# microsoft/ORBIT-Dataset

Measured on AMD Instinct MI355X. Metric: query frames/sec per task (224×224, 5-way ProtoNet) + frame accuracy vs ref, higher is better.
Workload: dtype f32

## Files before the change

### orbit-dataset_amd/csrc/pw_stream.hip

```cpp
#include <algorithm>
#include <type_traits>
#include "common.h"
#include "se_gate.h"

namespace orbit {

using f32x4 = __attribute__((ext_vector_type(4))) float;

struct PwsParams {
    const float* x;
    const float* w;
    float* y;
    const float* scale;
    const float* shift;
    const float* residual;
    const float* partial;
    const float *w1, *b1, *w2t, *b2;
    float* gate_out;
    float inv_hw;
    int KT, chunks, R, HW, Cout;
    int tiles;
    int bpf;
};

template <int KC, int NG, int TP>
__global__ __launch_bounds__(256) void pw_stream_kernel(PwsParams p) {
    constexpr int K = 16 * KC;
    extern __shared__ __attribute__((aligned(16))) float sm[];
    f32x4* wl = reinterpret_cast<f32x4*>(sm);
    float* gl = sm + KC * NG * 256;
    float* sg = gl + K;
    const int tid = threadIdx.x, lane = tid & 63, wave = tid >> 6;
    const int q = lane >> 4;
    const int b = blockIdx.x / p.bpf, seg = blockIdx.x - b * p.bpf;
    const int t_beg = (int)((long)seg * p.tiles / p.bpf), t_end = (int)((long)(seg + 1) * p.tiles / p.bpf);
    const size_t pix0 = (size_t)b * p.HW + (lane & 15);
    const bool has_res = p.residual != nullptr;

    auto has = [&](int s) { return t_beg + (4 * s + wave) * TP < t_end; };
    auto tile_of = [&](int s, int u) { return t_beg + (4 * s + wave) * TP + u; };
    auto row_of = [&](int s, int u) {
        const int t = tile_of(s, u);
        return pix0 + (size_t)16 * (t < t_end ? t : tile_of(s, 0));
    };

    f32x4 xa[TP][KC];
    if (has(0)) {
#pragma unroll
        for (int u = 0; u < TP; ++u) {
            const float* px = p.x + row_of(0, u) * K + 4 * q;
#pragma unroll
            for (int c = 0; c < KC; ++c) xa[u][c] = *reinterpret_cast<const f32x4*>(px + 16 * c);
        }
    }

    for (int i = tid; i < KC * NG * 64; i += 256) {
        const int l = i & 63, g = (i >> 6) % NG, c = (i >> 6) / NG;
        wl[i] = *reinterpret_cast<const f32x4*>(p.w + (size_t)(16 * g + (l & 15)) * p.KT + 16 * c + 4 * (l >> 4));
    }
    se_gate_frame<256, 4>(p.partial + (size_t)b * p.chunks * K, p.chunks, p.inv_hw, p.w1, p.b1, p.w2t, p.b2, gl, K, p.R,
                          nullptr, sg);
    __syncthreads();
    if (p.gate_out != nullptr && seg == 0)
        for (int c4 = tid; c4 < K / 4; c4 += 256)
            reinterpret_cast<f32x4*>(p.gate_out + (size_t)b * K)[c4] = reinterpret_cast<const f32x4*>(gl)[c4];

    f32x4 sc[NG], sh[NG];
#pragma unroll
    for (int g = 0; g < NG; ++g) {
        const int ch = 16 * g + 4 * q;
        const bool ok = ch < p.Cout;
        sc[g] = ok ? *reinterpret_cast<const f32x4*>(p.scale + ch) : (f32x4){0.f, 0.f, 0.f, 0.f};
        sh[g] = ok ? *reinterpret_cast<const f32x4*>(p.shift + ch) : (f32x4){0.f, 0.f, 0.f, 0.f};
    }

    auto step = [&](int s, auto refill) {
        constexpr bool REFILL = decltype(refill)::value;
        __asm__ volatile("" ::: "memory");
        size_t row[TP], nrow[TP];
#pragma unroll
        for (int u = 0; u < TP; ++u) row[u] = row_of(s, u), nrow[u] = REFILL ? row_of(s + 1, u) : row[u];
        f32x4 rr[TP][NG];
        if (has_res)
#pragma unroll
            for (int u = 0; u < TP; ++u)
#pragma unroll
                for (int g = 0; g < NG; ++g) {
                    const int ch = 16 * g + 4 * q;
                    rr[u][g] = *reinterpret_cast<const f32x4*>(p.residual + row[u] * p.Cout + (ch < p.Cout ? ch : 0));
                }
        f32x4 acc[TP][NG];
#pragma unroll
        for (int u = 0; u < TP; ++u)
#pragma unroll
            for (int g = 0; g < NG; ++g) acc[u][g] = (f32x4){0.f, 0.f, 0.f, 0.f};
#pragma unroll
        for (int c = 0; c < KC; ++c) {
            const f32x4 gv = *reinterpret_cast<const f32x4*>(gl + 16 * c + 4 * q);
            f32x4 xv[TP];
#pragma unroll
            for (int u = 0; u < TP; ++u) {
                xv[u] = xa[u][c] * gv;
                if (REFILL) xa[u][c] = *reinterpret_cast<const f32x4*>(p.x + nrow[u] * K + 4 * q + 16 * c);
            }
#pragma unroll
            for (int g = 0; g < NG; ++g) {
                const f32x4 wv = wl[(c * NG + g) * 64 + lane];
#pragma unroll
                for (int e = 0; e < 4; ++e)
#pragma unroll
                    for (int u = 0; u < TP; ++u)
                        acc[u][g] = __builtin_amdgcn_mfma_f32_16x16x4f32(wv[e], xv[u][e], acc[u][g], 0, 0, 0);
            }
        }
#pragma unroll
        for (int u = 0; u < TP; ++u) {
            if (tile_of(s, u) >= t_end) continue;
#pragma unroll
            for (int g = 0; g < NG; ++g) {
                const int ch = 16 * g + 4 * q;
                if (ch >= p.Cout) continue;
                f32x4 o = acc[u][g] * sc[g] + sh[g];
                if (has_res) o += rr[u][g];
                *reinterpret_cast<f32x4*>(p.y + row[u] * p.Cout + ch) = o;
            }
        }
    };
    int s = 0;
    for (; has(s + 1); ++s) step(s, std::true_type{});
    if (has(s)) step(s, std::false_type{});
}

namespace {
struct PwsVariant {
    int kc, ng, tp;
    void (*fn)(PwsParams);
};
const PwsVariant kVariants[] = {
    {2, 1, 2, pw_stream_kernel<2, 1, 2>},
    {6, 2, 1, pw_stream_kernel<6, 2, 1>},
    {9, 2, 1, pw_stream_kernel<9, 2, 1>},
    {9, 3, 1, pw_stream_kernel<9, 3, 1>},
};
const PwsVariant* find_variant(int Cin, int Cout) {
    if (Cin % 16 != 0 || Cout % 8 != 0 || Cout > 48) return nullptr;
    for (const PwsVariant& v : kVariants)
        if (v.kc == Cin / 16 && v.ng == cdiv(Cout, 16)) return &v;
    return nullptr;
}
}

bool pw_stream_supported(int Cin, int Cout, int H, int W) {
    return find_variant(Cin, Cout) != nullptr && (H * W) % 16 == 0;
}

int launch_pw_stream(const PwStreamDesc& d, hipStream_t s) {
    ORBIT_REQUIRE(d.x && d.w_packed && d.y && d.scale && d.shift && d.partial && d.w1 && d.b1 && d.w2t && d.b2,
                  "pw_stream: null pointer");
    ORBIT_REQUIRE(pw_stream_supported(d.Cin, d.Cout, d.H, d.W), "pw_stream: unsupported layer %d -> %d @%dx%d", d.Cin, d.Cout,
                  d.H, d.W);
    ORBIT_REQUIRE(d.B > 0 && d.chunks > 0 && d.se_hw > 0 && d.R > 0, "pw_stream: bad sizes");
    const PwsVariant& v = *find_variant(d.Cin, d.Cout);
    const ConvPackGeom geom = conv_pack_geom(d.Cin, d.Cout, 1, 1, 0);
    ORBIT_REQUIRE(geom.kt >= d.Cin && geom.cout_pad >= 16 * v.ng, "pw_stream: packed filter too small");
    PwsParams p;
    p.x = d.x, p.w = d.w_packed, p.y = d.y, p.scale = d.scale, p.shift = d.shift, p.residual = d.residual;
    p.partial = d.partial, p.w1 = d.w1, p.b1 = d.b1, p.w2t = d.w2t, p.b2 = d.b2, p.gate_out = d.gate_out;
    p.inv_hw = 1.0f / (float)d.se_hw;
    p.KT = geom.kt, p.chunks = d.chunks, p.R = d.R, p.HW = d.H * d.W, p.Cout = d.Cout;
    p.tiles = p.HW / 16;
    p.bpf = std::max(1, std::min(p.tiles, cdiv(p.tiles, 24 * v.tp)));
    ORBIT_REQUIRE((long long)d.B * p.bpf < (1ll << 31), "pw_stream: grid too large");
    const size_t lds = ((size_t)v.kc * v.ng * 256 + d.Cin + ((d.Cin + d.R + 3) & ~3) + 4 * 256) * sizeof(float);
    const double M = (double)d.B * p.HW;
    char name[48];
    snprintf(name, sizeof(name), "conv_pw_stream<%dx%d%s>", d.Cin, d.Cout, d.residual ? ",res" : "");
    const int rec = prof_start(name, 2.0 * M * d.Cin * d.Cout,
                               4.0 * (M * d.Cin + M * d.Cout * (d.residual ? 2.0 : 1.0) + (double)d.B * d.chunks * d.Cin), s);
    hipLaunchKernelGGL(v.fn, dim3((unsigned)(d.B * p.bpf)), dim3(256), lds, s, p);
    prof_stop(rec, s);
    ORBIT_LAUNCH_CHECK();
    return ORBIT_OK;
}

}

extern "C" {

int orbit_pw_stream_supported(int Cin, int Cout, int H, int W) { return orbit::pw_stream_supported(Cin, Cout, H, W) ? 1 : 0; }

int orbit_op_pw_stream(const float* x, const float* w, const float* scale, const float* shift, const float* residual,
                       const float* partial, int chunks, const float* w1, const float* b1, const float* w2t, const float* b2,
                       int R, float* y, float* gate_out, int B, int H, int W, int Cin, int Cout, orbit_stream_t stream) {
    using namespace orbit;
    ORBIT_REQUIRE(x && w && scale && shift && partial && w1 && b1 && w2t && b2 && y, "op_pw_stream: null pointer");
    hipStream_t s = (hipStream_t)stream;
    const bool fused = get_option("conv_rgemm") && pw_stream_supported(Cin, Cout, H, W);
    const size_t nfl = (conv_packed_floats(Cin, Cout, 1, 1, 0) + 63) & ~(size_t)63;
    const size_t ffl = conv_frag_floats(Cin, Cout, 1, 1, 0);
    const size_t gfl = (fused || gate_out) ? 0 : (size_t)B * Cin;
    float* wp = nullptr;
    ORBIT_HIP_CHECK(hipMallocAsync(reinterpret_cast<void**>(&wp), (nfl + ffl + gfl) * sizeof(float), s));
    int rc = conv_pack_weights(w, wp, Cin, Cout, 1, 1, 0, s);
    if (rc == ORBIT_OK && ffl) rc = conv_frag_pack_weights(w, wp + nfl, Cin, Cout, s);
    if (rc == ORBIT_OK && fused) {
        PwStreamDesc d;
        d.x = x, d.w_packed = wp, d.y = y, d.scale = scale, d.shift = shift, d.residual = residual;
        d.partial = partial, d.chunks = chunks, d.se_hw = H * W, d.w1 = w1, d.b1 = b1, d.w2t = w2t, d.b2 = b2, d.R = R;
        d.gate_out = gate_out, d.B = B, d.H = H, d.W = W, d.Cin = Cin, d.Cout = Cout;
        rc = launch_pw_stream(d, s);
    } else if (rc == ORBIT_OK) {
        float* gate = gate_out ? gate_out : wp + nfl + ffl;
        rc = launch_se_gate2(partial, chunks, H * W, w1, b1, w2t, b2, gate, B, Cin, R, s);
        if (rc == ORBIT_OK) {
            ConvDesc d;
            d.x = x, d.w_packed = wp, d.w_frag = ffl ? wp + nfl : nullptr, d.y = y, d.scale = scale, d.shift = shift;
            d.residual = residual, d.gate = gate, d.B = B, d.H = H, d.W = W, d.Cin = Cin, d.Cout = Cout, d.KH = d.KW = 1;
            d.stride = 1, d.pad_t = d.pad_l = 0, d.Ho = H, d.Wo = W, d.act = ORBIT_ACT_NONE, d.pool2 = 0, d.x_nchw = 0;
            rc = launch_conv(d, s);
        }
    }
    (void)hipFreeAsync(wp, s);
    return rc;
}

}
```

### orbit-dataset_amd/csrc/se_gate.h

```cpp
#pragma once
#include "common.h"
#include "device_util.h"

namespace orbit {

using v4f = __attribute__((ext_vector_type(4))) float;

template <int NT, int U>
__device__ __forceinline__ void se_gate_frame(const float* __restrict__ partial, int chunks, float inv_hw,
                                              const float* __restrict__ w1, const float* __restrict__ b1,
                                              const float* __restrict__ w2t, const float* __restrict__ b2,
                                              float* __restrict__ gate, int C, int R, float* __restrict__ pooled_out, float* sm2) {
    v4f* sp4 = reinterpret_cast<v4f*>(sm2);
    float* hid = sm2 + C;
    const int tid = threadIdx.x;
    const int C4 = C >> 2;
    const v4f* part4 = reinterpret_cast<const v4f*>(partial);
    const int parts = C4 <= NT / 2 ? NT / C4 : 1;
    if (parts > 1 && chunks > 8) {
        v4f* tmp = reinterpret_cast<v4f*>(sm2 + ((C + R + 3) & ~3));
        const int q = tid % C4, part = tid / C4;
        if (part < parts) {
            v4f s = {0.f, 0.f, 0.f, 0.f};
#pragma unroll 4
            for (int k = part; k < chunks; k += parts) s += part4[(size_t)k * C4 + q];
            tmp[part * C4 + q] = s;
        }
        __syncthreads();
        if (tid < C4) {
            v4f s = tmp[tid];
            for (int g = 1; g < parts; ++g) s += tmp[g * C4 + tid];
            sp4[tid] = s * inv_hw;
        }
    } else {
        for (int c4 = tid; c4 < C4; c4 += NT) {
            v4f s = {0.f, 0.f, 0.f, 0.f};
#pragma unroll 8
            for (int k = 0; k < chunks; ++k) s += part4[(size_t)k * C4 + c4];
            sp4[c4] = s * inv_hw;
        }
    }
    __syncthreads();
    if (pooled_out != nullptr)
        for (int c4 = tid; c4 < C4; c4 += NT) reinterpret_cast<v4f*>(pooled_out)[c4] = sp4[c4];
    const int lane = tid & 63, wave = tid >> 6;
    const v4f* w14 = reinterpret_cast<const v4f*>(w1);
    for (int r0 = wave; r0 < R; r0 += U * (NT / 64)) {
        float acc[U];
#pragma unroll
        for (int u = 0; u < U; ++u) acc[u] = 0.f;
        for (int cb = 0; cb < C4; cb += 320) {
            v4f wv[U][5], pv[5];
#pragma unroll
            for (int j = 0; j < 5; ++j) {
                const int c4 = cb + lane + 64 * j;
                const bool ok = c4 < C4;
                pv[j] = ok ? sp4[c4] : (v4f){0.f, 0.f, 0.f, 0.f};
#pragma unroll
                for (int u = 0; u < U; ++u) {
                    const int r = r0 + (NT / 64) * u;
                    wv[u][j] = (ok && r < R) ? w14[(size_t)r * C4 + c4] : (v4f){0.f, 0.f, 0.f, 0.f};
                }
            }
#pragma unroll
            for (int u = 0; u < U; ++u)
#pragma unroll
                for (int j = 0; j < 5; ++j) {
                    const v4f t = wv[u][j] * pv[j];
                    acc[u] += (t[0] + t[1]) + (t[2] + t[3]);
                }
        }
#pragma unroll
        for (int u = 0; u < U; ++u) {
            const int r = r0 + (NT / 64) * u;
            const float sum = wave_sum_dpp(acc[u]);
            if (r < R && lane == 0) {
                const float t = sum + b1[r];
                hid[r] = t / (1.0f + expf(-t));
            }
        }
    }
    __syncthreads();
    const v4f* w24 = reinterpret_cast<const v4f*>(w2t);
    for (int c4 = tid; c4 < C4; c4 += NT) {
        v4f a = *reinterpret_cast<const v4f*>(b2 + 4 * c4);
        int r = 0;
        for (; r + 8 <= R; r += 8) {
            v4f wv[8];
#pragma unroll
            for (int u = 0; u < 8; ++u) wv[u] = w24[(size_t)(r + u) * C4 + c4];
#pragma unroll
            for (int u = 0; u < 8; ++u) a += wv[u] * hid[r + u];
        }
        for (; r < R; ++r) a += w24[(size_t)r * C4 + c4] * hid[r];
        v4f g;
#pragma unroll
        for (int q = 0; q < 4; ++q) g[q] = 1.0f / (1.0f + expf(-a[q]));
        reinterpret_cast<v4f*>(gate)[c4] = g;
    }
}

}
```

Measured before the change: 37360.

## Issue pw_stream prologue loads early and pick blocks-per-frame from occupancy

```diff
diff --git a/orbit-dataset_amd/csrc/pw_stream.hip b/orbit-dataset_amd/csrc/pw_stream.hip
--- a/orbit-dataset_amd/csrc/pw_stream.hip
+++ b/orbit-dataset_amd/csrc/pw_stream.hip
@@ -23,13 +23,16 @@
     int bpf;
 };
 
+constexpr int pws_waves(int KC) { return KC == 2 ? 5 : 4; }
+
 template <int KC, int NG, int TP>
-__global__ __launch_bounds__(256) void pw_stream_kernel(PwsParams p) {
+__global__ __launch_bounds__(256) __attribute__((amdgpu_waves_per_eu(pws_waves(KC)))) void pw_stream_kernel(PwsParams p) {
     constexpr int K = 16 * KC;
     extern __shared__ __attribute__((aligned(16))) float sm[];
     f32x4* wl = reinterpret_cast<f32x4*>(sm);
     float* gl = sm + KC * NG * 256;
-    float* sg = gl + K;
+    f32x4* ssl = reinterpret_cast<f32x4*>(gl + K);
+    float* sg = gl + K + 32 * NG;
     const int tid = threadIdx.x, lane = tid & 63, wave = tid >> 6;
     const int q = lane >> 4;
     const int b = blockIdx.x / p.bpf, seg = blockIdx.x - b * p.bpf;
@@ -44,6 +47,17 @@
         return pix0 + (size_t)16 * (t < t_end ? t : tile_of(s, 0));
     };
 
+    constexpr int NW = (KC * NG * 64 + 255) / 256;
+    f32x4 wq[NW];
+#pragma unroll
+    for (int j = 0; j < NW; ++j) {
+        const int i = tid + 256 * j < KC * NG * 64 ? tid + 256 * j : 0;
+        const int l = i & 63, g = (i >> 6) % NG, c = (i >> 6) / NG;
+        wq[j] = *reinterpret_cast<const f32x4*>(p.w + (size_t)(16 * g + (l & 15)) * p.KT + 16 * c + 4 * (l >> 4));
+    }
+    const int sch = 4 * (tid % (4 * NG)) < p.Cout ? 4 * (tid % (4 * NG)) : 0;
+    const f32x4 ssq = *reinterpret_cast<const f32x4*>((tid < 4 * NG ? p.scale : p.shift) + sch);
+    const SeGateLoads<4> gq = se_gate_request<256, 4, K>(p.w1, p.b1, p.w2t, p.b2, p.R);
     f32x4 xa[TP][KC];
     if (has(0)) {
 #pragma unroll
@@ -53,26 +67,15 @@
             for (int c = 0; c < KC; ++c) xa[u][c] = *reinterpret_cast<const f32x4*>(px + 16 * c);
         }
     }
-
-    for (int i = tid; i < KC * NG * 64; i += 256) {
-        const int l = i & 63, g = (i >> 6) % NG, c = (i >> 6) / NG;
-        wl[i] = *reinterpret_cast<const f32x4*>(p.w + (size_t)(16 * g + (l & 15)) * p.KT + 16 * c + 4 * (l >> 4));
-    }
-    se_gate_frame<256, 4>(p.partial + (size_t)b * p.chunks * K, p.chunks, p.inv_hw, p.w1, p.b1, p.w2t, p.b2, gl, K, p.R,
-                          nullptr, sg);
+#pragma unroll
+    for (int j = 0; j < NW; ++j)
+        if (tid + 256 * j < KC * NG * 64) wl[tid + 256 * j] = wq[j];
+    if (tid < 8 * NG) ssl[tid] = ssq;
+    se_gate_frame_early<256, 4, K>(gq, p.partial + (size_t)b * p.chunks * K, p.chunks, p.inv_hw, gl, p.R, sg);
     __syncthreads();
     if (p.gate_out != nullptr && seg == 0)
         for (int c4 = tid; c4 < K / 4; c4 += 256)
             reinterpret_cast<f32x4*>(p.gate_out + (size_t)b * K)[c4] = reinterpret_cast<const f32x4*>(gl)[c4];
-
-    f32x4 sc[NG], sh[NG];
-#pragma unroll
-    for (int g = 0; g < NG; ++g) {
-        const int ch = 16 * g + 4 * q;
-        const bool ok = ch < p.Cout;
-        sc[g] = ok ? *reinterpret_cast<const f32x4*>(p.scale + ch) : (f32x4){0.f, 0.f, 0.f, 0.f};
-        sh[g] = ok ? *reinterpret_cast<const f32x4*>(p.shift + ch) : (f32x4){0.f, 0.f, 0.f, 0.f};
-    }
 
     auto step = [&](int s, auto refill) {
         constexpr bool REFILL = decltype(refill)::value;
@@ -120,7 +123,7 @@
             for (int g = 0; g < NG; ++g) {
                 const int ch = 16 * g + 4 * q;
                 if (ch >= p.Cout) continue;
-                f32x4 o = acc[u][g] * sc[g] + sh[g];
+                f32x4 o = acc[u][g] * ssl[4 * g + q] + ssl[4 * NG + 4 * g + q];
                 if (has_res) o += rr[u][g];
                 *reinterpret_cast<f32x4*>(p.y + row[u] * p.Cout + ch) = o;
             }
@@ -135,16 +138,45 @@
 struct PwsVariant {
     int kc, ng, tp;
     void (*fn)(PwsParams);
+    size_t occ_lds;
+    int occ;
 };
-const PwsVariant kVariants[] = {
-    {2, 1, 2, pw_stream_kernel<2, 1, 2>},
-    {6, 2, 1, pw_stream_kernel<6, 2, 1>},
-    {9, 2, 1, pw_stream_kernel<9, 2, 1>},
-    {9, 3, 1, pw_stream_kernel<9, 3, 1>},
+PwsVariant kVariants[] = {
+    {2, 1, 2, pw_stream_kernel<2, 1, 2>, 0, 0},
+    {6, 2, 1, pw_stream_kernel<6, 2, 1>, 0, 0},
+    {9, 2, 1, pw_stream_kernel<9, 2, 1>, 0, 0},
+    {9, 3, 1, pw_stream_kernel<9, 3, 1>, 0, 0},
 };
-const PwsVariant* find_variant(int Cin, int Cout) {
+
+long resident_blocks(PwsVariant& v, size_t lds) {
+    static int cus = 0;
+    if (v.occ_lds != lds || cus == 0) {
+        int dev = 0, n = 0;
+        if (hipGetDevice(&dev) != hipSuccess ||
+            hipDeviceGetAttribute(&cus, hipDeviceAttributeMultiprocessorCount, dev) != hipSuccess ||
+            hipOccupancyMaxActiveBlocksPerMultiprocessor(&n, v.fn, 256, lds) != hipSuccess)
+            return 0;
+        v.occ = n, v.occ_lds = lds;
+    }
+    return (long)v.occ * cus;
+}
+
+constexpr int kPrologueBytes = 20 * 1024;
+int blocks_per_frame(int B, int tiles, int K, int tp, long slots) {
+    const double pro = (double)kPrologueBytes / (64.0 * K);
+    int best = 1;
+    double best_cost = 0.0;
+    for (int bpf = 1; bpf <= tiles; ++bpf) {
+        const long rounds = ((long)B * bpf + slots - 1) / slots;
+        const double cost = (double)rounds * (pro + 4 * tp * cdiv(cdiv(tiles, bpf), 4 * tp));
+        if (bpf == 1 || cost < best_cost) best = bpf, best_cost = cost;
+    }
+    return best;
+}
+
+PwsVariant* find_variant(int Cin, int Cout) {
     if (Cin % 16 != 0 || Cout % 8 != 0 || Cout > 48) return nullptr;
-    for (const PwsVariant& v : kVariants)
+    for (PwsVariant& v : kVariants)
         if (v.kc == Cin / 16 && v.ng == cdiv(Cout, 16)) return &v;
     return nullptr;
 }
@@ -160,7 +192,9 @@
     ORBIT_REQUIRE(pw_stream_supported(d.Cin, d.Cout, d.H, d.W), "pw_stream: unsupported layer %d -> %d @%dx%d", d.Cin, d.Cout,
                   d.H, d.W);
     ORBIT_REQUIRE(d.B > 0 && d.chunks > 0 && d.se_hw > 0 && d.R > 0, "pw_stream: bad sizes");
-    const PwsVariant& v = *find_variant(d.Cin, d.Cout);
+    ORBIT_REQUIRE((se_gate_early_fits<256, 4>(d.Cin, d.R)), "pw_stream: %d hidden units do not fit the gate prologue at %d channels",
+                  d.R, d.Cin);
+    PwsVariant& v = *find_variant(d.Cin, d.Cout);
     const ConvPackGeom geom = conv_pack_geom(d.Cin, d.Cout, 1, 1, 0);
     ORBIT_REQUIRE(geom.kt >= d.Cin && geom.cout_pad >= 16 * v.ng, "pw_stream: packed filter too small");
     PwsParams p;
@@ -169,9 +203,11 @@
     p.inv_hw = 1.0f / (float)d.se_hw;
     p.KT = geom.kt, p.chunks = d.chunks, p.R = d.R, p.HW = d.H * d.W, p.Cout = d.Cout;
     p.tiles = p.HW / 16;
-    p.bpf = std::max(1, std::min(p.tiles, cdiv(p.tiles, 24 * v.tp)));
+    const size_t lds = ((size_t)v.kc * v.ng * 256 + d.Cin + 32 * v.ng + ((d.Cin + d.R + 3) & ~3) + 4 * 256) * sizeof(float);
+    const long slots = resident_blocks(v, lds);
+    ORBIT_REQUIRE(slots > 0, "pw_stream: occupancy query failed");
+    p.bpf = blocks_per_frame(d.B, p.tiles, d.Cin, v.tp, slots);
     ORBIT_REQUIRE((long long)d.B * p.bpf < (1ll << 31), "pw_stream: grid too large");
-    const size_t lds = ((size_t)v.kc * v.ng * 256 + d.Cin + ((d.Cin + d.R + 3) & ~3) + 4 * 256) * sizeof(float);
     const double M = (double)d.B * p.HW;
     char name[48];
     snprintf(name, sizeof(name), "conv_pw_stream<%dx%d%s>", d.Cin, d.Cout, d.residual ? ",res" : "");
diff --git a/orbit-dataset_amd/csrc/se_gate.h b/orbit-dataset_amd/csrc/se_gate.h
--- a/orbit-dataset_amd/csrc/se_gate.h
+++ b/orbit-dataset_amd/csrc/se_gate.h
@@ -100,4 +100,108 @@
     }
 }
 
-}
+template <int U>
+struct SeGateLoads {
+    v4f w1[U];
+    float b1[U];
+    v4f w2, b2;
+};
+
+template <int NT, int U>
+__host__ __device__ constexpr bool se_gate_early_fits(int C, int R) {
+    return C % 4 == 0 && C / 4 <= 64 && R <= U * (NT / 64) && R * (C / 4) <= NT;
+}
+
+template <int NT, int U, int C>
+__device__ __forceinline__ SeGateLoads<U> se_gate_request(const float* __restrict__ w1, const float* __restrict__ b1,
+                                                          const float* __restrict__ w2t, const float* __restrict__ b2, int R) {
+    constexpr int C4 = C >> 2;
+    static_assert(C % 4 == 0 && C4 <= 64, "se_gate_request: one channel quad per lane");
+    const int tid = threadIdx.x, lane = tid & 63, wave = tid >> 6;
+    SeGateLoads<U> g;
+#pragma unroll
+    for (int u = 0; u < U; ++u) {
+        const int r = wave + (NT / 64) * u, rc = r < R ? r : 0;
+        g.w1[u] = reinterpret_cast<const v4f*>(w1)[(size_t)rc * C4 + (lane < C4 ? lane : 0)];
+        g.b1[u] = b1[rc];
+    }
+    g.w2 = reinterpret_cast<const v4f*>(w2t)[tid < R * C4 ? tid : 0];
+    g.b2 = reinterpret_cast<const v4f*>(b2)[tid < C4 ? tid : 0];
+    return g;
+}
+
+template <int NT, int U, int C>
+__device__ __forceinline__ void se_gate_frame_early(const SeGateLoads<U>& g, const float* __restrict__ partial, int chunks,
+                                                    float inv_hw, float* __restrict__ gate, int R, float* sm2) {
+    constexpr int C4 = C >> 2;
+    v4f* sp4 = reinterpret_cast<v4f*>(sm2);
+    float* hid = sm2 + C;
+    v4f* tmp = reinterpret_cast<v4f*>(sm2 + ((C + R + 3) & ~3));
+    const int tid = threadIdx.x;
+    const v4f* part4 = reinterpret_cast<const v4f*>(partial);
+    constexpr int parts = C4 <= NT / 2 ? NT / C4 : 1;
+    constexpr int NB = parts >= 16 ? 4 : 8;
+    auto sum_chunks = [&](int k0, int stride, int q) {
+        v4f s = {0.f, 0.f, 0.f, 0.f};
+        for (int k = k0; k < chunks; k += NB * stride) {
+            v4f v[NB];
+#pragma unroll
+            for (int j = 0; j < NB; ++j) {
+                const int kk = k + j * stride;
+                v[j] = part4[(size_t)(kk < chunks ? kk : chunks - 1) * C4 + q];
+            }
+#pragma unroll
+            for (int j = 0; j < NB; ++j)
+                if (k + j * stride < chunks) s += v[j];
+        }
+        return s;
+    };
+    if (parts > 1 && chunks > 8) {
+        const int q = tid % C4, part = tid / C4;
+        if (part < parts) tmp[part * C4 + q] = sum_chunks(part, parts, q);
+        __syncthreads();
+        if (tid < C4) {
+            v4f s = tmp[tid];
+            for (int p = 1; p < parts; ++p) s += tmp[p * C4 + tid];
+            sp4[tid] = s * inv_hw;
+        }
+    } else if (tid < C4) {
+        sp4[tid] = sum_chunks(0, 1, tid) * inv_hw;
+    }
+    __syncthreads();
+    if (tid < R * C4) tmp[tid] = g.w2;
+    const int lane = tid & 63, wave = tid >> 6;
+    const v4f zero = {0.f, 0.f, 0.f, 0.f};
+    const v4f pv = lane < C4 ? sp4[lane] : zero;
+#pragma unroll
+    for (int u = 0; u < U; ++u) {
+        const int r = wave + (NT / 64) * u;
+        float acc = 0.f;
+        const v4f t = (lane < C4 ? g.w1[u] : zero) * pv;
+        acc += (t[0] + t[1]) + (t[2] + t[3]);
+        const float sum = wave_sum_dpp(acc);
+        if (r < R && lane == 0) {
+            const float h = sum + g.b1[u];
+            hid[r] = h / (1.0f + expf(-h));
+        }
+    }
+    __syncthreads();
+    if (tid < C4) {
+        v4f a = g.b2;
+        int r = 0;
+        for (; r + 8 <= R; r += 8) {
+            v4f wv[8];
+#pragma unroll
+            for (int u = 0; u < 8; ++u) wv[u] = tmp[(r + u) * C4 + tid];
+#pragma unroll
+            for (int u = 0; u < 8; ++u) a += wv[u] * hid[r + u];
+        }
+        for (; r < R; ++r) a += tmp[r * C4 + tid] * hid[r];
+        v4f o;
+#pragma unroll
+        for (int q = 0; q < 4; ++q) o[q] = 1.0f / (1.0f + expf(-a[q]));
+        reinterpret_cast<v4f*>(gate)[tid] = o;
+    }
+}
+
+}
```

Result: no change. 37400 (median of 6 runs) (+0.1%).
